# RainbowZL0/swin-unet-image-fusion

Hardware: AMD Instinct MI355X
Metric: fused image-pairs/sec at 256x256, win=8 (higher is better)
Workload: dtype bf16; 1 GPU; B=16/GPU 256x256 IR/visible pairs, win=8, 5-level Swin-UNet fusion forward (BASELINE configs[1]); global_batch=16, precision_mode=fast, residual_stream=fp32, hip_graph=True, steps_in_flight=3, kernel_schedule=throughput, collective=none, weights=random-init (numpy PCG64 recipe, seed 0)

## Files before the change

### swin_unet_image_fusion_amd/csrc/kernels_win24.hip

```cpp
#include "win_host.h"

namespace swf {
namespace {

using namespace wf;

constexpr int W24_WAVES = 3;

template <int HID_>
struct G24 {
    static constexpr int C = 24, HID = HID_, HEADS = 8, D = 3;
    static constexpr bool ONES_H = HID % 32 != 0;
    static constexpr int NT1 = (HID + (ONES_H ? 1 : 0) + 31) / 32;
    static constexpr int KU = (HID + (ONES_H ? 1 : 0) + 15) / 16;
    static constexpr int F_QKV = 0;
    static constexpr int F_P = 12;
    static constexpr int F_W1 = 16;
    static constexpr int F_W2 = F_W1 + 4 * NT1;
    static constexpr int NFRAG = F_W2 + 2 * KU;
    static constexpr size_t p_vec = size_t(NFRAG) * 1024;
    static constexpr int V_LN1G = 0, V_LN1B = 12, V_LN2G = 24, V_LN2B = 36, V_B2 = 48;
    static constexpr size_t p_bias = p_vec + 2 * 64 * 4;
    static constexpr size_t p_total = p_bias + size_t(2) * 2 * 16 * 64 * 4;
    static constexpr size_t l_k = 0, l_v = l_k + 16 * 1024, l_vec = l_v + 16 * 1024, l_zero = l_vec + 2 * 2 * 64 * 4,
                            l_total = l_zero + kPvZeroBytes;
    static constexpr size_t p_total16 = p_bias + size_t(15) * 64 * 16 * 4;
    static constexpr size_t l_k16 = 0, l_v16 = 32 * 1024, l_vec16 = 64 * 1024, l_zero16 = l_vec16 + 2 * 2 * 64 * 4, l_total16 = l_zero16 + kPvZeroBytes;
};

__device__ __forceinline__ void layernorm_frags(const f32x16& res, const float* vec, int goff, int boff, u32x4 (&xh)[2], u32x4 (&xl)[2]) {
    float s = 0.f;
#pragma unroll
    for (int i = 0; i < 12; ++i) s += res[i];
    const float mean = sum_halves(s) * (1.0f / 24.0f);
    float d[12], q = 0.f;
#pragma unroll
    for (int i = 0; i < 12; ++i) {
        d[i] = res[i] - mean;
        q += d[i] * d[i];
    }
    const float rstd = __builtin_amdgcn_rsqf(sum_halves(q) * (1.0f / 24.0f) + 1e-5f);
    float n[16];
#pragma unroll
    for (int a = 0; a < 3; ++a) {
        const float4 g = *reinterpret_cast<const float4*>(vec + goff + 4 * a);
        const float4 b = *reinterpret_cast<const float4*>(vec + boff + 4 * a);
        n[4 * a + 0] = d[4 * a + 0] * rstd * g.x + b.x;
        n[4 * a + 1] = d[4 * a + 1] * rstd * g.y + b.y;
        n[4 * a + 2] = d[4 * a + 2] * rstd * g.z + b.z;
        n[4 * a + 3] = d[4 * a + 3] * rstd * g.w + b.w;
    }
    n[12] = 1.0f;
    n[13] = n[14] = n[15] = 0.f;
    split8(n, xh[0], xl[0]);
    split8(n + 8, xh[1], xl[1]);
}

__device__ __forceinline__ void raw_frags(const f32x16& res, u32x4 (&xh)[2], u32x4 (&xl)[2]) {
    float n[16];
#pragma unroll
    for (int i = 0; i < 12; ++i) n[i] = res[i];
    n[12] = 1.0f;
    n[13] = n[14] = n[15] = 0.f;
    split8(n, xh[0], xl[0]);
    split8(n + 8, xh[1], xl[1]);
}

__device__ __forceinline__ const u32x4* pv_src24(const char* smem, int lane, unsigned vblk, unsigned zreg) {
    const unsigned off = pv_match(lane) ? vblk + (unsigned)(((lane & 32) + (lane & 3)) * 16) : zreg + (unsigned)kPvZeroBase;
    return reinterpret_cast<const u32x4*>(smem + off);
}

template <bool ONLINE>
__device__ __forceinline__ f32x16 attention24(const u32x4* ksrc, const u32x4* vsrc, const u32x4 (&qf)[2], const f32x16 (&bias)[2], bool half1,
                                            f32x16 o, float* mrun = nullptr) {
#pragma unroll
    for (int h = 0; h < 8; ++h) {
        const int s = h >> 2, sub = (h >> 1) & 1;
        const bool keep = half1 == ((h & 1) != 0);
        const u32x4 ka0 = ksrc[(0 * 2 + s) * 64], ka1 = ksrc[(1 * 2 + s) * 64];
        u32x4 qm = {0u, 0u, 0u, 0u};
        qm[2 * sub] = keep ? qf[s][2 * sub] : 0u;
        qm[2 * sub + 1] = keep ? qf[s][2 * sub + 1] : 0u;
        f32x16 s0 = mfma_f16(ka0, qm, bias[0]);
        f32x16 s1 = mfma_f16(ka1, qm, bias[1]);
        float mx = max3f(s0[0], s0[1], s1[0]);
        mx = max3f(mx, s1[1], s0[2]);
#pragma unroll
        for (int i = 3; i < 16; i += 2) mx = max3f(mx, s0[i], s0[i + 1 < 16 ? i + 1 : i]);
#pragma unroll
        for (int i = 2; i < 16; i += 2) mx = max3f(mx, s1[i], s1[i + 1]);
        mx = max_halves(mx);
        float alpha = 0.f;
        f16 nm = (f16)(-mx);
        if constexpr (ONLINE) {
            const float mold = mrun[h >> 1];
            nm = (f16)(-__builtin_fmaxf(mold, mx));
            const float mnew = -(float)nm;
            alpha = __builtin_amdgcn_exp2f(mold - mnew);
            mrun[h >> 1] = keep ? mnew : mold;
        }
        const unsigned nmb = keep ? (unsigned)__builtin_bit_cast(unsigned short, nm) : 0u;
        qm[2 * sub + 1] |= nmb << 16;
        s0 = mfma_f16(ka0, qm, bias[0]);
        s1 = mfma_f16(ka1, qm, bias[1]);
        f32x4 t;
#pragma unroll
        for (int ps = 0; ps < 4; ++ps) {
            float p[8];
#pragma unroll
            for (int j = 0; j < 8; ++j) p[j] = __builtin_amdgcn_exp2f((ps >> 1) ? s1[8 * (ps & 1) + j] : s0[8 * (ps & 1) + j]);
            const u32x4 pf = pack8_f16(p);
            const u32x4 va = vsrc[ps * 64 + h * 4];
            t = mfma16_f16(va, pf, ps == 0 ? f32x4{0.f, 0.f, 0.f, 0.f} : t);
            __builtin_amdgcn_sched_barrier(0);
        }
#pragma unroll
        for (int j = 0; j < 4; ++j) {
            const int i = 4 * (h >> 1) + j;
            o[i] = keep ? (ONLINE ? __builtin_fmaf(o[i], alpha, t[j]) : t[j]) : o[i];
        }
        __builtin_amdgcn_sched_barrier(0);
    }
    return o;
}

__device__ __forceinline__ void load_rows24(const __amdgpu_buffer_rsrc_t& irs, unsigned tokoff, f32x16& dstv) {
#pragma unroll
    for (int a = 0; a < 3; ++a) {
        const f32x4 v = __builtin_bit_cast(f32x4, __builtin_amdgcn_raw_buffer_load_b128(irs, tokoff, 32 * a, 0));
        dstv[4 * a] = v.x; dstv[4 * a + 1] = v.y; dstv[4 * a + 2] = v.z; dstv[4 * a + 3] = v.w;
    }
    dstv[12] = dstv[13] = dstv[14] = dstv[15] = 0.f;
}
__device__ __forceinline__ void store_rows24(__amdgpu_buffer_rsrc_t ors, unsigned tokoff, f32x16 res) {
#pragma unroll
    for (int a = 0; a < 3; ++a) {
        const f32x4 v = {res[4 * a], res[4 * a + 1], res[4 * a + 2], res[4 * a + 3]};
        __builtin_amdgcn_raw_buffer_store_b128(__builtin_bit_cast(u32x4, v), ors, tokoff, 32 * a, 0);
    }
}

template <class G, class WFn>
__device__ __forceinline__ f32x16 project24(WFn WF, f32x16 o, f32x16 res) {
    float t[16];
#pragma unroll
    for (int a = 0; a < 4; ++a) {
        const float inv = __builtin_amdgcn_rcpf(o[4 * a + 3]);
        t[4 * a] = o[4 * a] * inv; t[4 * a + 1] = o[4 * a + 1] * inv; t[4 * a + 2] = o[4 * a + 2] * inv;
        t[4 * a + 3] = 1.0f;
    }
    u32x4 oh[2], ol[2];
    split8(t, oh[0], ol[0]);
    split8(t + 8, oh[1], ol[1]);
    SWF_WF_FENCE();
#pragma unroll
    for (int s = 0; s < 2; ++s) res = mma3(WF(G::F_P + 2 * s), WF(G::F_P + 2 * s + 1), oh[s], ol[s], res);
    return res;
}


template <int HID, int WS, int MODE = WIN_BLOCK, bool RAW = false>
__global__ __launch_bounds__(256, W24_WAVES) void window24_kernel(WinArgs args) {
    using G = G24<HID>;
    static_assert(WS == 7 || WS == 8, "window side");
    static_assert(MODE == WIN_BLOCK || MODE == WIN_ATTN || MODE == WIN_MLP, "mode");
    static_assert(!RAW || MODE != WIN_BLOCK, "RAW belongs to the half-block modes");
    constexpr bool ATT = MODE != WIN_MLP, MLP = MODE != WIN_ATTN;
    __shared__ __attribute__((aligned(16))) char smem[G::l_total];
    u32x4* kimg = reinterpret_cast<u32x4*>(smem + G::l_k);
    u32x4* vimg = reinterpret_cast<u32x4*>(smem + G::l_v);
    float* lvec = reinterpret_cast<float*>(smem + G::l_vec);

    const int tid = threadIdx.x, lane = tid & 63, wave = tid >> 6;
    const int ws = wave >> 1, qb = wave & 1, r = lane & 31, hf = lane >> 5;
    const int H = args.H, W = args.W, nwx = MLP && !ATT ? 1 : W / WS, nwy = MLP && !ATT ? 1 : H / WS, npi = nwx * nwy;
    const int nwin = ATT ? args.B * npi : (max(args.ntok[0], args.ntok[1]) + 63) / 64;
    const int sh = args.shift ? WS / 2 : 0;
    const int kvs = args.cross ? 1 - ws : ws;

    for (int i = tid; i < 2 * 2 * 64; i += 256) lvec[i] = reinterpret_cast<const float*>(args.packed[i >> 7] + G::p_vec)[i & 127];
    const __amdgpu_buffer_rsrc_t wrs = __builtin_amdgcn_make_buffer_rsrc(const_cast<char*>(uniform_ptr(args.packed[ws])), 0, (int)G::p_total, 0x00020000);
    const __amdgpu_buffer_rsrc_t krs = __builtin_amdgcn_make_buffer_rsrc(const_cast<char*>(uniform_ptr(args.packed[kvs])), 0, (int)G::p_total, 0x00020000);
    const int act_bytes = ATT ? args.B * H * W * 24 * 4 : args.ntok[ws] * 24 * 4;
    const __amdgpu_buffer_rsrc_t irs = __builtin_amdgcn_make_buffer_rsrc(const_cast<float*>(uniform_ptr(args.in[ws])), 0, act_bytes, 0x00020000);
    const __amdgpu_buffer_rsrc_t ors = __builtin_amdgcn_make_buffer_rsrc(uniform_ptr(args.out[ws]), 0, (MODE == WIN_BLOCK || args.out[ws]) ? act_bytes : 0, 0x00020000);
    const unsigned loff = (unsigned)lane * 16u;
    auto WF = [&](int f) { return __builtin_bit_cast(u32x4, __builtin_amdgcn_raw_buffer_load_b128(wrs, loff, f * 1024, 0)); };
    auto WK = [&](int f) { return __builtin_bit_cast(u32x4, __builtin_amdgcn_raw_buffer_load_b128(krs, loff, f * 1024, 0)); };
    const float* vec = lvec + (ws * 2 + hf) * 64;
    f32x16 bias[2];
    auto load_bias = [&]() {
        const int vo = lane * 128 + qb * (2 * 16 * 64 * 4);
#pragma unroll
        for (int kt = 0; kt < 2; ++kt)
#pragma unroll
            for (int q4 = 0; q4 < 4; ++q4) {
                const f32x4 t = __builtin_bit_cast(f32x4, __builtin_amdgcn_raw_buffer_load_b128(wrs, vo + (kt * 16 + q4 * 4) * 4, (int)G::p_bias, 0));
#pragma unroll
                for (int e = 0; e < 4; ++e) bias[kt][q4 * 4 + e] = t[e];
            }
    };
    if constexpr (ATT) {
        load_bias();
        pv_fill_zeros<256>(smem + G::l_zero, tid);
    }
    const bool half1 = hf != 0;
    const bool col_masked = half1 != (((r >> 2) & 1) != 0);
    __syncthreads();

    int it = 0;
    for (int win = blockIdx.x; win < nwin; win += gridDim.x, ++it) {
        SWF_WF_FENCE();
        const int b = win / npi, wrem = win - b * npi;
        const int wy = wrem / nwx, wx = wrem - wy * nwx;
        const int buf = it & 1;
        int lane_w = lane;
        asm volatile("" : "+v"(lane_w));
        const int ty = 4 * qb + ((lane_w >> 3) & 3), tx = lane_w & 7;
        unsigned oy = wy * WS + ty + sh, ox = wx * WS + tx + sh;
        oy = oy < oy - (unsigned)H ? oy : oy - (unsigned)H;
        ox = ox < ox - (unsigned)W ? ox : ox - (unsigned)W;
        const unsigned tokoff = [&]() -> unsigned {
            if constexpr (ATT) {
                return (WS == 8 || (ty < WS && tx < WS)) ? (unsigned)((((b * H + (int)oy) * W + (int)ox) * 24 + 4 * (lane_w >> 5)) * 4) : 0x80000000u;
            } else {
                const int tok = 64 * win + 32 * qb + (lane_w & 31);
                return tok < args.ntok[ws] ? (unsigned)((tok * 24 + 4 * (lane_w >> 5)) * 4) : 0x80000000u;
            }
        }();
        const f32x16 zero16 = {0.f, 0.f, 0.f, 0.f, 0.f, 0.f, 0.f, 0.f, 0.f, 0.f, 0.f, 0.f, 0.f, 0.f, 0.f, 0.f};

        f32x16 res;
        if constexpr (ATT) {
        u32x4 qf[2];
        {
            load_rows24(irs, tokoff, res);
            u32x4 xh[2], xl[2];
            if constexpr (RAW) raw_frags(res, xh, xl);
            else layernorm_frags(res, vec, G::V_LN1G, G::V_LN1B, xh, xl);
            f32x16 acc = zero16;
            if (!(RAW && ws == 1)) {
#pragma unroll
                for (int s = 0; s < 2; ++s) acc = mma3(WF(G::F_QKV + 2 * s), WF(G::F_QKV + 2 * s + 1), xh[s], xl[s], acc);
                float t[16];
#pragma unroll
                for (int i = 0; i < 16; ++i) t[i] = acc[i];
                qf[0] = pack8_f16(t);
                qf[1] = pack8_f16(t + 8);
            }
            SWF_WF_FENCE();
            if (!(RAW && ws == 0)) {
                float t[16];
                acc = zero16;
#pragma unroll
                for (int s = 0; s < 2; ++s) acc = mma3(WK(G::F_QKV + 4 + 2 * s), WK(G::F_QKV + 5 + 2 * s), xh[s], xl[s], acc);
#pragma unroll
                for (int i = 0; i < 16; ++i) t[i] = acc[i];
                u32x4* kdst = kimg + (((buf * 2 + kvs) * 2 + qb) * 2) * 64 + lane;
                kdst[0] = pack8_f16(t);
                kdst[64] = pack8_f16(t + 8);
                SWF_WF_FENCE();
                acc = zero16;
#pragma unroll
                for (int s = 0; s < 2; ++s) acc = mma3(xh[s], xl[s], WK(G::F_QKV + 8 + 2 * s), WK(G::F_QKV + 9 + 2 * s), acc);
#pragma unroll
                for (int i = 0; i < 16; ++i) t[i] = acc[i];
                u32x4* vdst = vimg + ((buf * 2 + kvs) * 4 + 2 * qb) * 64 + lane;
                vdst[0] = pack8_f16(t);
                vdst[64] = pack8_f16(t + 8);
            }
        }
        __syncthreads();
        if (RAW && ws == 1) continue;

        f32x16 o;
        {
            const bool rowv = args.shift && wy == nwy - 1, colv = args.shift && wx == nwx - 1;
            const u32x4* ksrc = kimg + ((buf * 2 + ws) * 4) * 64 + lane;
            const u32x4* vsrc = pv_src24(smem, lane_w, (unsigned)(G::l_v + ((buf * 2 + ws) * 4) * 1024), (unsigned)G::l_zero);
            if (rowv || colv) {
                const float pen0 = ((rowv && qb == 1) || (colv && col_masked)) ? -INFINITY : 0.f;
                const float pen1 = ((rowv && qb == 0) || (colv && col_masked)) ? -INFINITY : 0.f;
#pragma unroll
                for (int i = 0; i < 16; ++i) { bias[0][i] += pen0; bias[1][i] += pen1; }
            }
            o = attention24<false>(ksrc, vsrc, qf, bias, half1, zero16);
            if (rowv || colv) load_bias();
        }

        SWF_WF_FENCE();
        if constexpr (RAW) res = zero16;
        res = project24<G>(WF, o, res);
        } else {
            load_rows24(irs, tokoff, res);
        }

        if constexpr (MLP) {
            u32x4 xh[2], xl[2];
            if constexpr (RAW) { raw_frags(res, xh, xl); res = zero16; }
            else layernorm_frags(res, vec, G::V_LN2G, G::V_LN2B, xh, xl);
#pragma unroll
            for (int tI = 0; tI < G::NT1; ++tI) {
                SWF_WF_FENCE();
                f32x16 acc = zero16;
#pragma unroll
                for (int s = 0; s < 2; ++s)
                    acc = mma3(WF(G::F_W1 + 4 * tI + 2 * s), WF(G::F_W1 + 4 * tI + 2 * s + 1), xh[s], xl[s], acc);
                float e[16];
                elu_tile(acc, e);
#pragma unroll
                for (int s2 = 0; s2 < 2; ++s2) {
                    const int u = 2 * tI + s2;
                    if (u < G::KU) {
                        u32x4 hh, hl;
                        split8(e + 8 * s2, hh, hl);
                        SWF_WF_FENCE();
                        res = mma3(WF(G::F_W2 + 2 * u), WF(G::F_W2 + 2 * u + 1), hh, hl, res);
                    }
                }
                __builtin_amdgcn_sched_barrier(0);
            }
            if constexpr (!G::ONES_H) {
#pragma unroll
                for (int a = 0; a < 3; ++a) {
                    const float4 b2 = *reinterpret_cast<const float4*>(vec + G::V_B2 + 4 * a);
                    res[4 * a] += b2.x; res[4 * a + 1] += b2.y; res[4 * a + 2] += b2.z; res[4 * a + 3] += b2.w;
                }
            }
        }

        store_rows24(ors, tokoff, res);
    }

    if (args.warm[0]) warm_next_block<256>(args, tid);
}

template <int HID>
__global__ __launch_bounds__(256, 2) void window24w16_kernel(WinArgs args) {
    using G = G24<HID>;
    extern __shared__ __attribute__((aligned(16))) char smem16[];
    u32x4* kimg = reinterpret_cast<u32x4*>(smem16 + G::l_k16);
    u32x4* vimg = reinterpret_cast<u32x4*>(smem16 + G::l_v16);
    float* lvec = reinterpret_cast<float*>(smem16 + G::l_vec16);

    const int tid = threadIdx.x, lane = tid & 63, wave = tid >> 6;
    const int ws = wave >> 1, pw = wave & 1, r = lane & 31, hf = lane >> 5;
    const int H = args.H, W = args.W, nwx = W / 16, nwy = H / 16, npi = nwx * nwy;
    const int nwin = args.B * npi;
    const int sh = args.shift ? 8 : 0;
    const int kvs = args.cross ? 1 - ws : ws;

    for (int i = tid; i < 2 * 2 * 64; i += 256) lvec[i] = reinterpret_cast<const float*>(args.packed[i >> 7] + G::p_vec)[i & 127];
    const __amdgpu_buffer_rsrc_t wrs = __builtin_amdgcn_make_buffer_rsrc(const_cast<char*>(uniform_ptr(args.packed[ws])), 0, (int)G::p_total16, 0x00020000);
    const __amdgpu_buffer_rsrc_t krs = __builtin_amdgcn_make_buffer_rsrc(const_cast<char*>(uniform_ptr(args.packed[kvs])), 0, (int)G::p_total16, 0x00020000);
    const int act_bytes = args.B * H * W * 24 * 4;
    const __amdgpu_buffer_rsrc_t irs = __builtin_amdgcn_make_buffer_rsrc(const_cast<float*>(uniform_ptr(args.in[ws])), 0, act_bytes, 0x00020000);
    const __amdgpu_buffer_rsrc_t ors = __builtin_amdgcn_make_buffer_rsrc(uniform_ptr(args.out[ws]), 0, act_bytes, 0x00020000);
    const unsigned loff = (unsigned)lane * 16u;
    auto WF = [&](int f) { return __builtin_bit_cast(u32x4, __builtin_amdgcn_raw_buffer_load_b128(wrs, loff, f * 1024, 0)); };
    auto WK = [&](int f) { return __builtin_bit_cast(u32x4, __builtin_amdgcn_raw_buffer_load_b128(krs, loff, f * 1024, 0)); };
    const float* vec = lvec + (ws * 2 + hf) * 64;
    const bool half1 = hf != 0;
    const f32x16 zero16 = {0.f, 0.f, 0.f, 0.f, 0.f, 0.f, 0.f, 0.f, 0.f, 0.f, 0.f, 0.f, 0.f, 0.f, 0.f, 0.f};
    pv_fill_zeros<256>(smem16 + G::l_zero16, tid);
    __syncthreads();

    for (int win = blockIdx.x; win < nwin; win += gridDim.x) {
        SWF_WF_FENCE();
        const int b = win / npi, wrem = win - b * npi;
        const int wy = wrem / nwx, wx = wrem - wy * nwx;
        auto tokoff_of = [&](int j) {
            int lane_w = lane;
            asm volatile("" : "+v"(lane_w));
            unsigned oy = wy * 16 + 2 * j + ((lane_w >> 4) & 1) + sh, ox = wx * 16 + (lane_w & 15) + sh;
            oy = oy < oy - (unsigned)H ? oy : oy - (unsigned)H;
            ox = ox < ox - (unsigned)W ? ox : ox - (unsigned)W;
            return (unsigned)((((b * H + (int)oy) * W + (int)ox) * 24 + 4 * (lane_w >> 5)) * 4);
        };

        u32x4 qf[4][2];
#pragma unroll
        for (int q = 0; q < 4; ++q) { qf[q][0] = u32x4{0u, 0u, 0u, 0u}; qf[q][1] = u32x4{0u, 0u, 0u, 0u}; }
        {
            u32x4 wq[4], wk[4], wv[4];
#pragma unroll
            for (int i = 0; i < 4; ++i) { wq[i] = WF(G::F_QKV + i); wk[i] = WK(G::F_QKV + 4 + i); wv[i] = WK(G::F_QKV + 8 + i); }
#pragma unroll 1
            for (int jj = 0; jj < 4; ++jj) {
                const int j = 4 * pw + jj;
                f32x16 x0;
                load_rows24(irs, tokoff_of(j), x0);
                u32x4 xh[2], xl[2];
                layernorm_frags(x0, vec, G::V_LN1G, G::V_LN1B, xh, xl);
                f32x16 acc = zero16;
#pragma unroll
                for (int s = 0; s < 2; ++s) acc = mma3(wq[2 * s], wq[2 * s + 1], xh[s], xl[s], acc);
                float t[16];
#pragma unroll
                for (int i = 0; i < 16; ++i) t[i] = acc[i];
#pragma unroll
                for (int q = 0; q < 3; ++q) { qf[q][0] = qf[q + 1][0]; qf[q][1] = qf[q + 1][1]; }
                qf[3][0] = pack8_f16(t);
                qf[3][1] = pack8_f16(t + 8);
                acc = zero16;
#pragma unroll
                for (int s = 0; s < 2; ++s) acc = mma3(wk[2 * s], wk[2 * s + 1], xh[s], xl[s], acc);
#pragma unroll
                for (int i = 0; i < 16; ++i) t[i] = acc[i];
                u32x4* kdst = kimg + ((kvs * 8 + j) * 2) * 64 + lane;
                kdst[0] = pack8_f16(t);
                kdst[64] = pack8_f16(t + 8);
                acc = zero16;
#pragma unroll
                for (int s = 0; s < 2; ++s) acc = mma3(xh[s], xl[s], wv[2 * s], wv[2 * s + 1], acc);
#pragma unroll
                for (int i = 0; i < 16; ++i) t[i] = acc[i];
                u32x4* vdst = vimg + (kvs * 16 + 2 * j) * 64 + lane;
                vdst[0] = pack8_f16(t);
                vdst[64] = pack8_f16(t + 8);
            }
        }
        __syncthreads();

        const bool rowv = args.shift && wy == nwy - 1, colv = args.shift && wx == nwx - 1;
        const u32x4* ksrc = kimg + (ws * 16) * 64 + lane;
#pragma unroll 1
        for (int jj = 0; jj < 4; ++jj) {
            const int j = 4 * pw + jj;
            const unsigned tokoff = tokoff_of(j);
            f32x16 o = zero16;
            float mrun[4] = {-INFINITY, -INFINITY, -INFINITY, -INFINITY};
#pragma unroll 1
            for (int c = 0; c < 4; ++c) {
                if (rowv && ((j < 4) != (c < 2))) continue;
                f32x16 bias[2];
                {
                    const int d0 = __builtin_amdgcn_readfirstlane(2 * c - j + 7);
#pragma unroll
                    for (int kt = 0; kt < 2; ++kt)
#pragma unroll
                        for (int q4 = 0; q4 < 4; ++q4) {
                            const f32x4 tb = __builtin_bit_cast(f32x4, __builtin_amdgcn_raw_buffer_load_b128(wrs, lane * 64 + q4 * 16, (int)G::p_bias + (d0 + kt) * 4096, 0));
#pragma unroll
                            for (int e = 0; e < 4; ++e) bias[kt][q4 * 4 + e] = tb[e];
                        }
                    if (colv) col_seam16(bias, r);
                }
                const u32x4* vsrc = pv_src24(smem16, lane, (unsigned)(G::l_v16 + (ws * 16 + 4 * c) * 1024), (unsigned)G::l_zero16);
                o = attention24<true>(ksrc + (2 * c) * 2 * 64, vsrc, qf[0], bias, half1, o, mrun);
            }
#pragma unroll
            for (int q = 0; q < 3; ++q) { qf[q][0] = qf[q + 1][0]; qf[q][1] = qf[q + 1][1]; }

            f32x16 res;
            SWF_WF_FENCE();
            load_rows24(irs, tokoff, res);
            res = project24<G>(WF, o, res);
            u32x4 xh[2], xl[2];
            layernorm_frags(res, vec, G::V_LN2G, G::V_LN2B, xh, xl);
#pragma unroll
            for (int tI = 0; tI < G::NT1; ++tI) {
                SWF_WF_FENCE();
                f32x16 acc = zero16;
#pragma unroll
                for (int s = 0; s < 2; ++s)
                    acc = mma3(WF(G::F_W1 + 4 * tI + 2 * s), WF(G::F_W1 + 4 * tI + 2 * s + 1), xh[s], xl[s], acc);
                float e[16];
                elu_tile(acc, e);
#pragma unroll
                for (int s2 = 0; s2 < 2; ++s2) {
                    const int u = 2 * tI + s2;
                    if (u < G::KU) {
                        u32x4 hh, hl;
                        split8(e + 8 * s2, hh, hl);
                        SWF_WF_FENCE();
                        res = mma3(WF(G::F_W2 + 2 * u), WF(G::F_W2 + 2 * u + 1), hh, hl, res);
                    }
                }
                __builtin_amdgcn_sched_barrier(0);
            }
            if constexpr (!G::ONES_H) {
#pragma unroll
                for (int a = 0; a < 3; ++a) {
                    const float4 b2 = *reinterpret_cast<const float4*>(vec + G::V_B2 + 4 * a);
                    res[4 * a] += b2.x; res[4 * a + 1] += b2.y; res[4 * a + 2] += b2.z; res[4 * a + 3] += b2.w;
                }
            }
            store_rows24(ors, tokoff, res);
        }
        __syncthreads();
    }
}

template <int HID>
__global__ __launch_bounds__(256) void pack24_kernel(WinPackArgs a) {
    using G = G24<HID>;
    const int s = blockIdx.y;
    const swf_block_stream_params& p = a.p[s];
    char* dst = a.dst[s];
    const int gtid = blockIdx.x * blockDim.x + threadIdx.x, gsz = gridDim.x * blockDim.x;
    const float qscale = kLog2e / sqrtf(3.0f);
    auto lin = [](const swf_linear& l, int n, int k, int ld) { return pack_wgt(l, n * ld + k); };

    for (int idx = gtid; idx < G::NFRAG * 512; idx += gsz) {
        const int f = idx >> 9, lane = (idx >> 3) & 63, e = idx & 7;
        const int r = lane & 31, hf = lane >> 5;
        float val = 0.f;
        int hl;
        if (f < G::F_P) {
            const int t = f >> 2, st = (f >> 1) & 1;
            hl = f & 1;
            const int k = rho(8 * st + e, hf), head = r >> 2, c = r & 3;
            const swf_linear& l = t == 0 ? p.attn.q : t == 1 ? p.attn.k : p.attn.v;
            if (c < 3) {
                const int row = 3 * head + c;
                val = k < 24 ? lin(l, row, k, 24) : (k == 24 ? pack_bia(l, row) : 0.f);
                if (t == 0) val *= qscale;
            } else if (t != 0 && k == 24) {
                val = 1.0f;
            }
        } else if (f < G::F_W1) {
            const int st = ((f - G::F_P) >> 1) & 1;
            hl = f & 1;
            const int k = rho(8 * st + e, hf), head = k >> 2, c = k & 3;
            if (r < 24) val = c < 3 ? lin(p.attn.proj, r, 3 * head + c, 24) : (k == 3 ? pack_bia(p.attn.proj, r) : 0.f);
        } else if (f < G::F_W2) {
            const int g = f - G::F_W1, t = g >> 2, st = (g >> 1) & 1;
            hl = g & 1;
            const int k = rho(8 * st + e, hf), hid = 32 * t + r;
            if (hid < HID) val = (k < 24 ? lin(p.fc1, hid, k, 24) : (k == 24 ? pack_bia(p.fc1, hid) : 0.f)) * kLog2e;
            else if (G::ONES_H && hid == HID && k == 24) val = 1.0f;
        } else {
            const int g = f - G::F_W2, u = g >> 1;
            hl = g & 1;
            const int hid = 32 * (u >> 1) + rho(8 * (u & 1) + e, hf);
            if (r < 24) val = hid < HID ? lin(p.fc2, r, hid, HID) * kLn2 : ((G::ONES_H && hid == HID) ? pack_bia(p.fc2, r) : 0.f);
        }
        const bf16 hi = (bf16)val;
        reinterpret_cast<bf16*>(dst)[idx] = hl ? (bf16)(val - (float)hi) : hi;
    }
    float* vec = reinterpret_cast<float*>(dst + G::p_vec);
    for (int i = gtid; i < 128; i += gsz) {
        const int hf = i >> 6, j = i & 63, which = j / 12, k = j % 12;
        const int c = 8 * (k >> 2) + 4 * hf + (k & 3);
        float v = 0.f;
        if (which == 0) v = p.ln1.gamma ? p.ln1.gamma[c] : 1.f;
        else if (which == 1) v = p.ln1.beta ? p.ln1.beta[c] : 0.f;
        else if (which == 2) v = p.ln2.gamma ? p.ln2.gamma[c] : 1.f;
        else if (which == 3) v = p.ln2.beta ? p.ln2.beta[c] : 0.f;
        else if (which == 4) v = (p.fc2.weight && p.fc2.bias) ? p.fc2.bias[c] : 0.f;
        vec[i] = v;
    }
    if (p.attn.bias_table) pack_rel_bias<true>(reinterpret_cast<float*>(dst + G::p_bias), p.attn.bias_table, a.ws, gtid, gsz);
}

struct L24 {
    static constexpr int C = 24, D = 3, HID_WIDE = 96, HID_NARROW = 4, PACK_GRID = 32, WAVES = W24_WAVES;
    static constexpr const char *name = "win24", *pack_name = "pack_win24";
    template <int HID> using G = G24<HID>;
    template <int HID>
    static void pack(dim3 grid, const WinPackArgs& a, hipStream_t stream) { hipLaunchKernelGGL((pack24_kernel<HID>), grid, dim3(256), 0, stream, a); }
    template <int HID, int WS, int MODE, bool RAW>
    static int launch(const swf_block_desc&, const WinArgs& a, int grid, hipStream_t stream, int*) {
        hipLaunchKernelGGL((window24_kernel<HID, WS, MODE, RAW>), dim3(grid), dim3(256), 0, stream, a);
        return check_launch(MODE == WIN_BLOCK ? "window24" : "window24 (half block)");
    }
    template <int HID>
    static int launch16(const WinArgs& a, int nwin, hipStream_t stream) {
        constexpr int lds = (int)G24<HID>::l_total16;
        SWF_TRY(raise_lds_limit<&window24w16_kernel<HID>>(lds, "window24w16"));
        hipLaunchKernelGGL((window24w16_kernel<HID>), dim3(std::min(nwin, 2 * num_cus())), dim3(256), lds, stream, a);
        return check_launch("window24w16");
    }
};

}

const WinLevel& win24_level() {
    static const WinLevel level = win_level<L24>();
    return level;
}

}
```

Before: 9250 pairs/s.

## Prefetch next window's input rows into registers during current window compute

Computes the token offsets for the next window a block will process and issues its row loads early. The loads go out after the QKV stage barrier, or at loop start in MLP-only mode, so global-memory latency overlaps attention, projection and MLP work. The first window's rows are loaded before the bias and LN vector setup. This costs an extra f32x16 of live registers per thread, which may lower occupancy or cause spills under the 3-wave launch bound.

```diff
diff --git a/swin_unet_image_fusion_amd/csrc/kernels_win24.hip b/swin_unet_image_fusion_amd/csrc/kernels_win24.hip
--- a/swin_unet_image_fusion_amd/csrc/kernels_win24.hip
+++ b/swin_unet_image_fusion_amd/csrc/kernels_win24.hip
@@ -179,7 +179,6 @@
     const int sh = args.shift ? WS / 2 : 0;
     const int kvs = args.cross ? 1 - ws : ws;
 
-    for (int i = tid; i < 2 * 2 * 64; i += 256) lvec[i] = reinterpret_cast<const float*>(args.packed[i >> 7] + G::p_vec)[i & 127];
     const __amdgpu_buffer_rsrc_t wrs = __builtin_amdgcn_make_buffer_rsrc(const_cast<char*>(uniform_ptr(args.packed[ws])), 0, (int)G::p_total, 0x00020000);
     const __amdgpu_buffer_rsrc_t krs = __builtin_amdgcn_make_buffer_rsrc(const_cast<char*>(uniform_ptr(args.packed[kvs])), 0, (int)G::p_total, 0x00020000);
     const int act_bytes = ATT ? args.B * H * W * 24 * 4 : args.ntok[ws] * 24 * 4;
@@ -201,41 +200,57 @@
                 for (int e = 0; e < 4; ++e) bias[kt][q4 * 4 + e] = t[e];
             }
     };
-    if constexpr (ATT) {
-        load_bias();
-        pv_fill_zeros<256>(smem + G::l_zero, tid);
-    }
+    int wy_n = 0, wx_n = 0;
+    auto tok_of = [&](int w) -> unsigned {
+        int lane_w = lane;
+        asm volatile("" : "+v"(lane_w));
+        if constexpr (ATT) {
+            const int b = w / npi, wrem = w - b * npi;
+            const int wy = wrem / nwx, wx = wrem - wy * nwx;
+            wy_n = wy; wx_n = wx;
+            const int ty = 4 * qb + ((lane_w >> 3) & 3), tx = lane_w & 7;
+            unsigned oy = wy * WS + ty + sh, ox = wx * WS + tx + sh;
+            oy = oy < oy - (unsigned)H ? oy : oy - (unsigned)H;
+            ox = ox < ox - (unsigned)W ? ox : ox - (unsigned)W;
+            return (w < nwin && (WS == 8 || (ty < WS && tx < WS))) ? ((((unsigned)(b * H) + oy) * (unsigned)W + ox) * 24u + 4u * (unsigned)(lane_w >> 5)) * 4u : 0x80000000u;
+        } else {
+            const int tok = 64 * w + 32 * qb + (lane_w & 31);
+            return (w < nwin && tok < args.ntok[ws]) ? (unsigned)((tok * 24 + 4 * (lane_w >> 5)) * 4) : 0x80000000u;
+        }
+    };
+    f32x16 nxt;
+    unsigned tokoff_n = tok_of(blockIdx.x);
+    load_rows24(irs, tokoff_n, nxt);
+    SWF_WF_FENCE();
+    if constexpr (ATT) load_bias();
+    for (int i = tid; i < 2 * 2 * 64; i += 256) lvec[i] = reinterpret_cast<const float*>(args.packed[i >> 7] + G::p_vec)[i & 127];
+    if constexpr (ATT) pv_fill_zeros<256>(smem + G::l_zero, tid);
     const bool half1 = hf != 0;
     const bool col_masked = half1 != (((r >> 2) & 1) != 0);
     __syncthreads();
+    auto prefetch_rows = [&](int w) {
+        SWF_WF_FENCE();
+        tokoff_n = tok_of(w);
+        load_rows24(irs, tokoff_n, nxt);
+        SWF_WF_FENCE();
+        __builtin_amdgcn_sched_barrier(0);
+    };
+    const int gstep = gridDim.x;
 
     int it = 0;
-    for (int win = blockIdx.x; win < nwin; win += gridDim.x, ++it) {
+    for (int win = blockIdx.x; win < nwin; win += gstep, ++it) {
         SWF_WF_FENCE();
-        const int b = win / npi, wrem = win - b * npi;
-        const int wy = wrem / nwx, wx = wrem - wy * nwx;
+        const int wy = wy_n, wx = wx_n;
         const int buf = it & 1;
         int lane_w = lane;
         asm volatile("" : "+v"(lane_w));
-        const int ty = 4 * qb + ((lane_w >> 3) & 3), tx = lane_w & 7;
-        unsigned oy = wy * WS + ty + sh, ox = wx * WS + tx + sh;
-        oy = oy < oy - (unsigned)H ? oy : oy - (unsigned)H;
-        ox = ox < ox - (unsigned)W ? ox : ox - (unsigned)W;
-        const unsigned tokoff = [&]() -> unsigned {
-            if constexpr (ATT) {
-                return (WS == 8 || (ty < WS && tx < WS)) ? (unsigned)((((b * H + (int)oy) * W + (int)ox) * 24 + 4 * (lane_w >> 5)) * 4) : 0x80000000u;
-            } else {
-                const int tok = 64 * win + 32 * qb + (lane_w & 31);
-                return tok < args.ntok[ws] ? (unsigned)((tok * 24 + 4 * (lane_w >> 5)) * 4) : 0x80000000u;
-            }
-        }();
+        const unsigned tokoff = tokoff_n;
         const f32x16 zero16 = {0.f, 0.f, 0.f, 0.f, 0.f, 0.f, 0.f, 0.f, 0.f, 0.f, 0.f, 0.f, 0.f, 0.f, 0.f, 0.f};
 
-        f32x16 res;
+        f32x16 res = nxt;
         if constexpr (ATT) {
         u32x4 qf[2];
         {
-            load_rows24(irs, tokoff, res);
             u32x4 xh[2], xl[2];
             if constexpr (RAW) raw_frags(res, xh, xl);
             else layernorm_frags(res, vec, G::V_LN1G, G::V_LN1B, xh, xl);
@@ -272,6 +287,7 @@
             }
         }
         __syncthreads();
+        prefetch_rows(win + gstep);
         if (RAW && ws == 1) continue;
 
         f32x16 o;
@@ -293,7 +309,7 @@
         if constexpr (RAW) res = zero16;
         res = project24<G>(WF, o, res);
         } else {
-            load_rows24(irs, tokoff, res);
+            prefetch_rows(win + gstep);
         }
 
         if constexpr (MLP) {
```

New measurement: 9300 pairs/s, median of 3. No clear change (+0.5%).
